# omid-arhami/topolow

Hardware: AMD Instinct MI355X
Metric: relaxation iterations/sec (NxN pairs) (higher is better)
Workload: dtype f32

## Files before the change

### topolow_amd/csrc/relax_symm.h

```cpp
#pragma once

#include <hip/hip_runtime.h>
#include <algorithm>
#include <type_traits>
#include <vector>
#include "relax_common.h"

namespace topolow {

#ifndef TOPOLOW_SYM_MINW
#define TOPOLOW_SYM_MINW 2
#endif
constexpr int kSymRows = 64;
constexpr int kSymCols = 32;
constexpr int kSymTileWords = kSymRows * kSymCols;
constexpr int kSymWaves = 4;

template <int DIM> struct SymRec { static constexpr int W = (DIM + 2 + 3) & ~3; };

struct SymUnit {
  int tile_row;
  int j0, j1;
  int tile0;
};

TL_HD inline long long sym_tile_index(int R, int J, int TC) { return (long long)R * TC - (long long)R * (R - 1) + (J - 2 * R); }
TL_HD inline size_t sym_word_in_tile(int r, int c) {
  const int a = r >> 3, p = (r & 7) >> 1, e = r & 1, b = c >> 2, h = (c & 3) >> 1, f = c & 1;
  return (size_t)((((4 * h + p) * 64) + a + 8 * b) * 4 + 2 * (f ^ (a & 1)) + e);
}

struct SymRun {
  int u0, u1;
  SymUnit first;
};
struct SymPlan {
  std::vector<SymUnit> units;
  std::vector<int> wave_first;
  std::vector<int2> row_units;
  std::vector<SymRun> runs() const {
    std::vector<SymRun> r(wave_first.size() - 1);
    for (size_t w = 0; w + 1 < wave_first.size(); ++w) {
      r[w].u0 = wave_first[w];
      r[w].u1 = wave_first[w + 1];
      r[w].first = r[w].u0 < r[w].u1 ? units[r[w].u0] : SymUnit{0, 0, 0, 0};
    }
    return r;
  }
};
inline SymPlan relax_symm_plan(int npad, int n_waves, long long t0 = 0, long long t1 = -1, int* r_first = nullptr,
                               int* r_last = nullptr) {
  SymPlan P;
  const int TR = npad / kSymRows, TC = npad / kSymCols;
  if (t1 < 0) t1 = (long long)TR * (TR + 1);
  const long long total = t1 - t0;
  int rf = -1, rl = -1;
  for (int R = 0; R < TR; ++R) {
    const long long a = sym_tile_index(R, 2 * R, TC), b = a + (TC - 2 * R);
    if (b > t0 && a < t1) { if (rf < 0) rf = R; rl = R; }
  }
  if (r_first) *r_first = rf;
  if (r_last) *r_last = rl;
  P.wave_first.assign(n_waves + 1, 0);
  if (rf < 0) return P;
  P.row_units.resize(rl - rf + 1);
  long long done = 0;
  int w = 0;
  long long w_end = (total * (w + 1) + n_waves - 1) / n_waves;
  for (int R = rf; R <= rl; ++R) {
    P.row_units[R - rf].x = (int)P.units.size();
    const long long row0 = sym_tile_index(R, 2 * R, TC);
    int j = 2 * R + (int)std::max<long long>(0, t0 - row0);
    const int j_end = 2 * R + (int)std::min<long long>(TC - 2 * R, t1 - row0);
    while (j < j_end) {
      while (done >= w_end && w + 1 < n_waves) {
        ++w;
        P.wave_first[w] = (int)P.units.size();
        w_end = (total * (w + 1) + n_waves - 1) / n_waves;
// ... 113 lines not shown
  bool sp0, sp1;
  if constexpr (THR) {
    const symf2 e0 = t - r;
    auto decide = [](uint32_t w, float e) {
      const uint32_t flip = (w << 30) & 0x80000000u;
      const int32_t some = (int32_t)(((w >> 1) | w) << 31) >> 31;
      const uint32_t q = ((f32_bits(e) ^ flip) & (uint32_t)some) | (0x3f800000u & ~(uint32_t)some);
      return bits_f32(q) > 0.0f;
    };
    sp0 = decide(w0, e0.x);
    sp1 = decide(w1, e0.y);
  } else {
    sp0 = __builtin_amdgcn_classf(bits_f32(w0), 0x1f8);
    sp1 = __builtin_amdgcn_classf(bits_f32(w1), 0x1f8);
  }
  const symf2 e = t - r;
  const symf2 inv2 = inv * inv;
  const symf2 u = {sp0 ? e.x : inv2.x, sp1 ? e.y : inv2.y};
  const symf2 base = u * inv;
  const symf2 mr = {sp0 ? ks2.x : cg2.x, sp1 ? ks2.y : cg2.y};
  const symf2 coef = base * mr;
#pragma unroll
  for (int d = 0; d < DIM; ++d) racc2[d] = __builtin_elementwise_fma(dx[d], coef, racc2[d]);
  const symf2 mc = {sp0 ? ksc : cgc, sp1 ? ksc : cgc};
  const symf2 cc = base * mc;
#pragma unroll
  for (int d = 0; d < DIM; ++d)
    cacc2[d] = FIRST ? dx[d] * cc : __builtin_elementwise_fma(dx[d], cc, cacc2[d]);
  if constexpr (ERR) {
    const symf2 a = {sp0 ? fabsf(e.x) : 0.0f, sp1 ? fabsf(e.y) : 0.0f};
    err2 += a;
    if constexpr (CNT) cnt_wave += (sp0 ? 1u : 0u) + (sp1 ? 1u : 0u);
  }
}

template <int DIM, bool ANYTHR, bool ERR>
__global__ __launch_bounds__(64 * kSymWaves, TOPOLOW_SYM_MINW) void symm_sweep_kernel(
    const uint32_t* __restrict__ enc, const float* __restrict__ rec, const SymUnit* __restrict__ units,
    const SymRun* __restrict__ runs, float* __restrict__ rowpart, float* __restrict__ colpart, int npad,
    const RunState* st, double* __restrict__ part_sum, unsigned long long* __restrict__ part_cnt,
    unsigned long long fixed_cnt, int col_row0) {
  if (st != nullptr && st->stopped) return;
#ifdef TOPOLOW_SYM_STAMPS
  const unsigned long long stamp_c0 = __builtin_amdgcn_s_memtime(), stamp_r0 = __builtin_amdgcn_s_memrealtime();
#endif
  constexpr int W = SymRec<DIM>::W;
  constexpr int kRecVec = W / 4;
  constexpr int kTileVec = kSymCols * kRecVec;
  constexpr int kLdsVec = kTileVec + kSymCols / 4;
  __shared__ uint4 lds[kSymWaves][2][kLdsVec];
  auto lds_slot = [](int q) { return q + (q / (4 * kRecVec)); };
  const int lane = threadIdx.x & 63;
  const int wave = __builtin_amdgcn_readfirstlane(threadIdx.x >> 6);
  const int a = lane & 7, b = lane >> 3;

  const int gw = blockIdx.x * kSymWaves + wave;
  const SymRun run = runs[gw];
  const int u_begin = __builtin_amdgcn_readfirstlane(run.u0);
  const int u_end = __builtin_amdgcn_readfirstlane(run.u1);
  typedef unsigned int u32x4 __attribute__((ext_vector_type(4)));
  const __amdgpu_buffer_rsrc_t rec_rsrc = __builtin_amdgcn_make_buffer_rsrc(const_cast<float*>(rec), 0, npad * W * 4, 0x00020000);
  for (int u = u_begin; u < u_end; ++u) {
    const SymUnit U = u == u_begin ? run.first : units[u];
    const int R = __builtin_amdgcn_readfirstlane(U.tile_row);
    const int J0 = __builtin_amdgcn_readfirstlane(U.j0), J1 = __builtin_amdgcn_readfirstlane(U.j1);
    const int slot = u;
    const int tile0 = __builtin_amdgcn_readfirstlane(U.tile0);

    symf2 pi2[4][DIM], ks2[4], cg2[4], racc2[4][DIM];
    {
      const uint4* rr = reinterpret_cast<const uint4*>(rec + (size_t)(R * kSymRows + 8 * a) * W);
#pragma unroll
      for (int p = 0; p < 4; ++p) {
        float f[2][W];
#pragma unroll
        for (int e = 0; e < 2; ++e)
#pragma unroll
          for (int v = 0; v < kRecVec; ++v) {
            const uint4 q = rr[(2 * p + e) * kRecVec + v];
            f[e][4 * v + 0] = __builtin_bit_cast(float, q.x);
            f[e][4 * v + 1] = __builtin_bit_cast(float, q.y);
            f[e][4 * v + 2] = __builtin_bit_cast(float, q.z);
            f[e][4 * v + 3] = __builtin_bit_cast(float, q.w);
          }
#pragma unroll
        for (int d = 0; d < DIM; ++d) {
          pi2[p][d] = (symf2){f[0][d], f[1][d]};
          racc2[p][d] = (symf2){0.0f, 0.0f};
        }
        ks2[p] = (symf2){f[0][DIM], f[1][DIM]};
        cg2[p] = (symf2){f[0][DIM + 1], f[1][DIM + 1]};
      }
    }
    const __amdgpu_buffer_rsrc_t rsrc = __builtin_amdgcn_make_buffer_rsrc(
        const_cast<uint32_t*>(enc) + (size_t)tile0 * kSymTileWords, 0, (J1 - J0) * kSymTileWords * 4, 0x00020000);
    const __amdgpu_buffer_rsrc_t col_rsrc = __builtin_amdgcn_make_buffer_rsrc(colpart + (size_t)(R - col_row0) * npad * DIM, 0, npad * DIM * 4, 0x00020000);
    const int col_off = a < 2 ? (4 * b + a) * DIM * 4 : 0x40000000;
    const int swap = a & 1;
    auto request = [&](int J, int h, u32x4 (&dst)[4]) {
#pragma unroll
      for (int p = 0; p < 4; ++p)
        dst[p] = __builtin_amdgcn_raw_buffer_load_b128(rsrc, lane * 16 + ((J - J0) * 8 + 4 * h + p) * 1024, 0, 0);
    };
    u32x4 wa[4], wb[4];
    request(J0, 0, wa);
    const uint4* recv = reinterpret_cast<const uint4*>(rec);
    if (lane < kTileVec) lds[wave][J0 & 1][lds_slot(lane)] = recv[(size_t)J0 * kTileVec + lane];
    if constexpr (kTileVec > 64) if (lane + 64 < kTileVec) lds[wave][J0 & 1][lds_slot(lane + 64)] = recv[(size_t)J0 * kTileVec + lane + 64];

    symf2 err2 = {0.0f, 0.0f};
    float err_unit = 0.0f;
    unsigned cnt_wave = 0, cnt_unit2 = 0;
    auto read_rec = [&](int J, int idx, float (&f)[W]) {
      const int col = idx ^ swap;
      const uint4* cp = &lds[wave][J & 1][4 * b * kRecVec + b];
#pragma unroll
      for (int v = 0; v < kRecVec; ++v) {
        const uint4 q = cp[col * kRecVec + v];
        f[4 * v + 0] = __builtin_bit_cast(float, q.x);
        f[4 * v + 1] = __builtin_bit_cast(float, q.y);
        f[4 * v + 2] = __builtin_bit_cast(float, q.z);
        f[4 * v + 3] = __builtin_bit_cast(float, q.w);
      }
    };
    float f_first[W];
    read_rec(J0, 0, f_first);
#pragma unroll 1
    for (int J = J0; J < J1; ++J) {
      const int Jn = J + 1 < J1 ? J + 1 : J;
      request(J, 1, wb);
      u32x4 rn0 = {0, 0, 0, 0}, rn1 = {0, 0, 0, 0};
      rn0 = __builtin_amdgcn_raw_buffer_load_b128(rec_rsrc, (Jn * kTileVec + lane) * 16, 0, 0);
      if constexpr (kTileVec > 64) rn1 = __builtin_amdgcn_raw_buffer_load_b128(rec_rsrc, (Jn * kTileVec + lane + 64) * 16, 0, 0);
      __builtin_amdgcn_sched_barrier(0);

      const bool diag = J < 2 * R + 2;
      float fq[4][W];
#pragma unroll
      for (int q = 0; q < W; ++q) fq[0][q] = f_first[q];
      auto half = [&](auto hc, const u32x4 (&wc)[4]) {
        constexpr int h = decltype(hc)::value;
        symf2 cacc2[2][DIM];
#pragma unroll
        for (int c = 0; c < 2; ++c) {
          if (2 * h + c + 1 < 4) {
            read_rec(J, 2 * h + c + 1, fq[2 * h + c + 1]);
            __builtin_amdgcn_sched_barrier(0);
          }
          const float (&f)[W] = fq[2 * h + c];
          float pc[DIM];
#pragma unroll
          for (int d = 0; d < DIM; ++d) pc[d] = f[d];
          const float ksc = f[DIM], cgc = f[DIM + 1];
#pragma unroll
          for (int p = 0; p < 4; ++p) {
            const uint32_t w0 = c == 0 ? wc[p].x : wc[p].z, w1 = c == 0 ? wc[p].y : wc[p].w;
            if (p == 0)
              sym_pair<DIM, ANYTHR, ERR, ANYTHR, true>(pc, ksc, cgc, pi2[p], ks2[p], cg2[p], w0, w1, racc2[p], cacc2[c], err2, cnt_wave);
            else
              sym_pair<DIM, ANYTHR, ERR, ANYTHR, false>(pc, ksc, cgc, pi2[p], ks2[p], cg2[p], w0, w1, racc2[p], cacc2[c], err2, cnt_wave);
          }
// ... 60 lines not shown
#pragma unroll
      for (int m = 32; m >= 1; m >>= 1) s += __shfl_xor(s, m, 64);
      if constexpr (ANYTHR) {
#pragma unroll
        for (int m = 32; m >= 1; m >>= 1) cnt_unit2 += __shfl_xor(cnt_unit2, m, 64);
      }
      if (lane == 0) {
        part_sum[slot] = s;
        part_cnt[slot] = ANYTHR ? (unsigned long long)cnt_unit2 : (slot == 0 ? fixed_cnt : 0ull);
      }
    }
  }
#ifdef TOPOLOW_SYM_STAMPS
  if (lane == 0 && g_sym_stamps != nullptr) {
    g_sym_stamps[4 * gw] = __builtin_amdgcn_s_memtime() - stamp_c0;
    g_sym_stamps[4 * gw + 1] = stamp_r0;
    g_sym_stamps[4 * gw + 2] = __builtin_amdgcn_s_memrealtime();
    unsigned hw_id, xcc_id;
    asm volatile("s_getreg_b32 %0, hwreg(HW_REG_HW_ID)" : "=s"(hw_id));
    asm volatile("s_getreg_b32 %0, hwreg(HW_REG_XCC_ID)" : "=s"(xcc_id));
    g_sym_stamps[4 * gw + 3] = ((unsigned long long)xcc_id << 32) | hw_id;
  }
#endif
}

template <int DIM, typename real> struct SymReal;
template <int DIM> struct SymReal<DIM, float> {
  static constexpr int W = SymRec<DIM>::W;
  __device__ static float ks(double k, float g) { return (float)(2.0 * k) / (4.0f * g + (float)k); }
  __device__ static float cg(double c_rep, float g) { return (float)(0.5 * c_rep) / g; }
  __device__ static float far(int) { return kFarF32; }
};

#ifndef TL_APPLY_PARTS
#define TL_APPLY_PARTS 16
#endif
constexpr int kSymApplyParts = TL_APPLY_PARTS;
template <int DIM, typename real>
__global__ __launch_bounds__(32 * kSymApplyParts) void symm_apply_kernel(
    const real* __restrict__ rec, real* __restrict__ rec_next, real* __restrict__ pos_out, const float* __restrict__ gplus,
    const real* __restrict__ rowpart, const real* __restrict__ colpart, const int2* __restrict__ row_units, int n,
    int npad, double k_next, double c_rep, int iter1, RunState* st, int rr_stages = 0, int rr_stage = 0) {
  if (st != nullptr && st->stopped) return;
  using T = SymReal<DIM, real>;
  constexpr int W = T::W;
  constexpr int kWavesA = kSymApplyParts / 2;
  __shared__ real red[kWavesA][kSymCols][DIM];
  const int R = blockIdx.x >> 1;
  const int part = threadIdx.x >> 5, pt = threadIdx.x & 31;
  const int i = blockIdx.x * kSymCols + pt;
  real acc[DIM];
#pragma unroll
  for (int d = 0; d < DIM; ++d) acc[d] = 0;
  int rp0 = 0, rp1 = R;
  if (rr_stages > 0) sym_rr_above(npad / kSymRows, rr_stages, rr_stage, R, rp0, rp1);
  for (int Rp = rp0 + part; Rp < rp1; Rp += kSymApplyParts) {
    const real* src = colpart + ((size_t)Rp * npad + i) * DIM;
#pragma unroll
    for (int d = 0; d < DIM; ++d) acc[d] += src[d];
  }
  const int2 ru = row_units[R];
  const int row_in_tile = i - R * kSymRows;
  for (int q = part; q < ru.y; q += kSymApplyParts) {
    const real* src = rowpart + ((size_t)(ru.x + q) * kSymRows + row_in_tile) * DIM;
#pragma unroll
    for (int d = 0; d < DIM; ++d) acc[d] -= src[d];
  }
#pragma unroll
  for (int d = 0; d < DIM; ++d) {
    if constexpr (std::is_same<real, float>::value) acc[d] += __shfl_xor(acc[d], 32, 64);
    else acc[d] += T::lane_xor(acc[d], 32);
  }
  const int wave = threadIdx.x >> 6;
  if ((threadIdx.x & 32) == 0) {
#pragma unroll
    for (int d = 0; d < DIM; ++d) red[wave][pt][d] = acc[d];
  }
  __syncthreads();
  if (part == 0 && i < n) {
    bool finite = true;
    real out[DIM];
#pragma unroll
    for (int d = 0; d < DIM; ++d) {
      real t = red[0][pt][d];
#pragma unroll
      for (int p = 1; p < kWavesA; ++p) t += red[p][pt][d];
      out[d] = rec[(size_t)i * W + d] + t;
      finite = finite && isfinite(out[d]);
      pos_out[(size_t)i * DIM + d] = out[d];
      rec_next[(size_t)i * W + d] = out[d];
    }
    const real g = (real)gplus[i];
    rec_next[(size_t)i * W + DIM] = T::ks(k_next, g);
    rec_next[(size_t)i * W + DIM + 1] = T::cg(c_rep, g);
    if (!finite && st != nullptr) atomicMin(&st->first_nonfinite, iter1);
  }
}

template <int DIM, typename real>
__global__ __launch_bounds__(256) void symm_records_kernel(const real* __restrict__ pos, const float* __restrict__ gplus,
                                                          real* __restrict__ rec, int n, int npad, double k, double c_rep) {
  using T = SymReal<DIM, real>;
  constexpr int W = T::W;
  const int i = blockIdx.x * blockDim.x + threadIdx.x;
  if (i >= npad) return;
  real* r = rec + (size_t)i * W;
  if (i < n) {
#pragma unroll
    for (int d = 0; d < DIM; ++d) r[d] = pos[(size_t)i * DIM + d];
    const real g = (real)gplus[i];
    r[DIM] = T::ks(k, g);
    r[DIM + 1] = T::cg(c_rep, g);
  } else {
#pragma unroll
    for (int d = 0; d < DIM; ++d) r[d] = T::far(d);
    r[DIM] = 0;
    r[DIM + 1] = 0;
  }
#pragma unroll
  for (int d = DIM + 2; d < W; ++d) r[d] = 0;
}

__global__ __launch_bounds__(256) void symm_tiles_kernel(const uint32_t* const* __restrict__ src, const int* __restrict__ row0,
                                                        int n_src, int ld, uint32_t* __restrict__ tenc, int TC,
                                                        long long t_first) {
  const long long t = t_first + blockIdx.x;
  int R = 0;
  {
    const double b = (double)TC + 1.0;
    const double disc = b * b - 4.0 * (double)t;
    R = (int)((b - sqrt(disc > 0.0 ? disc : 0.0)) * 0.5);
    while (R > 0 && (long long)R * TC - (long long)R * (R - 1) > t) --R;
    while ((long long)(R + 1) * TC - (long long)(R + 1) * R <= t) ++R;
  }
  const int J = 2 * R + (int)(t - ((long long)R * TC - (long long)R * (R - 1)));
  uint32_t* dst = tenc + (size_t)blockIdx.x * kSymTileWords;
  const int rows = row0[n_src];
#pragma unroll
  for (int q = 0; q < kSymTileWords / 256; ++q) {
    const int cell = threadIdx.x + q * 256;
    const int r = cell >> 5, c = cell & 31;
    const int row = R * kSymRows + r, col = J * kSymCols + c;
    uint32_t w = kInfWord;
    if (row < rows && col < ld) {
      int blk = 0;
      while (blk + 1 < n_src && row >= row0[blk + 1]) ++blk;
      w = src[blk][enc_index(row - row0[blk], col, ld)];
    }
    const int a = r >> 3, p = (r & 7) >> 1, e = r & 1, b = c >> 2, h = (c & 3) >> 1, f = c & 1;
    dst[(((4 * h + p) * 64) + a + 8 * b) * 4 + 2 * (f ^ (a & 1)) + e] = w;
  }
}


template <int DIM>
__global__ __launch_bounds__(32 * 32) void symm_partial_kernel(
    const float* __restrict__ rowpart, const float* __restrict__ colpart, const int2* __restrict__ row_units, int r_first,
    int r_last, int n, int npad, float* const* __restrict__ inbox, const int* __restrict__ own0, int n_own, int slot,
    const RunState* st) {
  if (st != nullptr && st->stopped) return;
  __shared__ float red[32][kSymCols][DIM];
  const int R = blockIdx.x >> 1;
  const int part = threadIdx.x >> 5, pt = threadIdx.x & 31;
  const int i = blockIdx.x * kSymCols + pt;
  float acc[DIM];
#pragma unroll
  for (int d = 0; d < DIM; ++d) acc[d] = 0.0f;
  const int r_stop = R < r_last + 1 ? R : r_last + 1;
  for (int Rp = r_first + part; Rp < r_stop; Rp += 32) {
    const float* src = colpart + ((size_t)(Rp - r_first) * npad + i) * DIM;
#pragma unroll
    for (int d = 0; d < DIM; ++d) acc[d] += src[d];
  }
  if (R >= r_first && R <= r_last) {
    const int2 ru = row_units[R - r_first];
    const int row_in_tile = i - R * kSymRows;
    for (int q = part; q < ru.y; q += 32) {
      const float* src = rowpart + ((size_t)(ru.x + q) * kSymRows + row_in_tile) * DIM;
#pragma unroll
      for (int d = 0; d < DIM; ++d) acc[d] -= src[d];
    }
  }
#pragma unroll
  for (int d = 0; d < DIM; ++d) red[part][pt][d] = acc[d];
  __syncthreads();
  if (part == 0 && i < n) {
    int q = 0;
    while (q + 1 < n_own && i >= own0[q + 1]) ++q;
    float* dst = inbox[q] + ((size_t)slot * npad + i) * DIM;
#pragma unroll
    for (int d = 0; d < DIM; ++d) {
      float t = red[0][pt][d];
#pragma unroll
      for (int p = 1; p < 32; ++p) t += red[p][pt][d];
      dst[d] = t;
    }
  }
}

template <int DIM>
__global__ __launch_bounds__(256) void symm_owner_apply_kernel(
    const float* __restrict__ pos_in, float* __restrict__ pos_out, const float* __restrict__ inbox, int n_slots, int npad,
    int row_begin, int row_end, float* const* __restrict__ push, int n_push, int iter1, RunState* st) {
  if (st != nullptr && st->stopped) return;
  const int i = row_begin + blockIdx.x * blockDim.x + threadIdx.x;
  if (i >= row_end) return;
  bool finite = true;
  float out[DIM];
#pragma unroll
  for (int d = 0; d < DIM; ++d) {
    float t = 0.0f;
    for (int b = 0; b < n_slots; ++b) t += inbox[((size_t)b * npad + i) * DIM + d];
    out[d] = pos_in[(size_t)i * DIM + d] + t;
    finite = finite && isfinite(out[d]);
    pos_out[(size_t)i * DIM + d] = out[d];
  }
  for (int q = 0; q < n_push; ++q) {
    float* dst = push[q];
#pragma unroll
// ... 7 lines not shown
```

### topolow_amd/csrc/topolow_relax.hip

```cpp

#include <hip/hip_runtime.h>

#include <chrono>
#include <cstdarg>
#include <cstdio>
#include <algorithm>
#include <cstring>
#include <cstdlib>
#include <array>
#include <atomic>
#include <deque>
#include <mutex>
#include <string>
#include <memory>
#include <thread>
#include <vector>

#include "../../include/topolow_relax.h"
#include "relax_common.h"
#include "relax_host.h"
#include "relax_kernels.h"
#include "relax_fold.h"
#include "relax_gs.h"
#include "relax_tilegs.h"
// ... 144 lines not shown
  struct SymState {
    bool allowed = false;
    int min_n = 0;
    bool ready = false;
    int npad = 0, tiles = 0, grid = 0;
    DevBuf<uint32_t> tenc;
    DevBuf<unsigned char> rec[2], rowpart, colpart;
    int rec_cur = 0, rec_iter = -1;
    DevBuf<float> tdelta;
    bool delta_ready = false;
    struct Plan {
      DevBuf<SymUnit> units;
      DevBuf<SymRun> runs;
      DevBuf<int2> row_units;
      int n_units = 0;
      void load(const SymPlan& hp) {
        const std::vector<SymRun> hr = hp.runs();
        n_units = (int)hp.units.size();
        units.alloc(std::max<size_t>(hp.units.size(), 1));
        runs.alloc(hr.size());
        row_units.alloc(std::max<size_t>(hp.row_units.size(), 1));
        if (!hp.units.empty())
          HIP_TRY(hipMemcpy(units.p, hp.units.data(), hp.units.size() * sizeof(SymUnit), hipMemcpyHostToDevice));
        HIP_TRY(hipMemcpy(runs.p, hr.data(), hr.size() * sizeof(SymRun), hipMemcpyHostToDevice));
        if (!hp.row_units.empty())
          HIP_TRY(hipMemcpy(row_units.p, hp.row_units.data(), hp.row_units.size() * sizeof(int2), hipMemcpyHostToDevice));
      }
      void release() { units.release(); runs.release(); row_units.release(); n_units = 0; }
    };
    Plan plan;
    std::vector<Plan> rr[4];
    bool whole = false;
    bool two_stage = true;
    int rr_min_tiles = 5;
    DevBuf<const uint32_t*> src_tab;
    DevBuf<int> src_row0;
    bool seg_ready = false;
    bool seg_thr = false;
    int seg_first = 0, seg_last = -1;
    int seg_slots = 0;
    int seg_slot = 0;
    bool seg_caller = false;
    DevBuf<float> inbox;
    DevBuf<float*> inbox_tab;
    DevBuf<int> own0;
    std::vector<const void*> seg_peers;

    void release() {
      tenc.release(); rec[0].release(); rec[1].release(); rowpart.release(); colpart.release();
      tdelta.release(); delta_ready = false;
      plan.release();
      for (auto& v : rr) v.clear();
      src_tab.release(); src_row0.release();
      inbox.release(); inbox_tab.release(); own0.release();
    }
  } sym;
  int fused_parts = 0;
  bool profiling = false;
  std::vector<std::pair<hipEvent_t, hipEvent_t>> prof_stage, prof_stage_err, prof_check;
  std::vector<std::pair<hipEvent_t, hipEvent_t>> prof_sym, prof_sym_err;

  size_t real_size() const { return precision == TOPOLOW_PRECISION_F64 ? 8 : 4; }
  int rows() const { return row_end - row_begin; }
  int pos_rows() const { return (n + 3) & ~3; }

  ~topolow_session() {
// ... 484 lines not shown
}

template <int DIM>
void sym_prepare(topolow_session* s) {
  sym_build<DIM>(s, {s->enc.p}, {0, s->rows()}, s->any_threshold, 0, -1);
  s->sym.ready = true;
  s->sym.seg_ready = false;
}

bool sym_available(topolow_session* s) {
  if (s->sym.ready) return true;
  try {
    TL_DISPATCH_SYM(s->dim, sym_prepare, s);
  } catch (const HipError&) {
    (void)hipGetLastError();
    s->sym.release();
    s->sym.ready = false;
    s->sym.allowed = false;
  }
  return s->sym.ready;
}

template <int DIM>
void sym_records(topolow_session* s, const void* pin, void* rec, double k) {
  sym_real(s, [&](auto r) {
    using real = decltype(r);
    hipLaunchKernelGGL((symm_records_kernel<DIM, real>), dim3((s->sym.npad + 255) / 256), dim3(256), 0, s->stream,
                       (const real*)pin, s->gplus.p, (real*)rec, s->n, s->sym.npad, k, s->c_rep);
  });
}

template <int DIM>
void sym_sweep(topolow_session* s, const SymPlanDev& plan, const void* rec, bool thr, bool err,
               unsigned long long block_cells, int col_row0) {
  auto& y = s->sym;
  sym_real(s, [&](auto r) {
    using real = decltype(r);
    sym_sweep_instance<DIM, real>(thr, err, [&](auto kern) {
      if constexpr (std::is_same<real, double>::value)
        hipLaunchKernelGGL(kern, dim3(y.grid), dim3(64 * kSymWaves), 0, s->stream, y.tenc.p, (const double*)rec,
                           plan.units.p, plan.runs.p, (double*)y.rowpart.p, (double*)y.colpart.p, y.npad, s->state.p,
                           col_row0, y.tdelta.p, s->part_sum.p, s->part_cnt.p, block_cells);
      else
        hipLaunchKernelGGL(kern, dim3(y.grid), dim3(64 * kSymWaves), 0, s->stream, y.tenc.p, (const float*)rec,
                           plan.units.p, plan.runs.p, (float*)y.rowpart.p, (float*)y.colpart.p, y.npad, s->state.p,
                           s->part_sum.p, s->part_cnt.p, block_cells, col_row0);
    });
  });
}

template <int DIM>
void sym_apply(topolow_session* s, const SymPlanDev& plan, const void* rec, void* rec_next, void* pout, double k_next,
               int iter, int rr_stages, int rr_stage) {
  auto& y = s->sym;
  sym_real(s, [&](auto r) {
    using real = decltype(r);
    hipLaunchKernelGGL((symm_apply_kernel<DIM, real>), dim3(y.npad / kSymCols), dim3(32 * kSymApplyParts), 0, s->stream,
                       (const real*)rec, (real*)rec_next, (real*)pout, s->gplus.p, (const real*)y.rowpart.p,
                       (const real*)y.colpart.p, plan.row_units.p, s->n, y.npad, k_next, s->c_rep, iter + 1, s->state.p,
                       rr_stages, rr_stage);
  });
}

bool sym_rr_stages_ok(int S) { return S == 2 || S == 4 || S == 8; }
int sym_rr_log2(int S) { return S == 2 ? 1 : (S == 4 ? 2 : 3); }

bool sym_rr_available(topolow_session* s, int S) {
  auto& y = s->sym;
  if (!sym_rr_stages_ok(S) || !y.whole) return false;
  const int TR = y.npad / kSymRows;
  if (TR < 2 * S) return false;
  if ((long long)TR * (TR + 1) / S < (long long)y.rr_min_tiles * y.grid * kSymWaves) return false;
  const int lg = sym_rr_log2(S);
  if (!y.rr[lg].empty()) return true;
  std::vector<SymPlanDev> plans(S);
  for (int st = 0; st < S; ++st) {
    const SymPlan hp = relax_symm_plan_rows(y.npad, y.grid * kSymWaves, [&](int R, int& j0, int& j1) { sym_rr_row(TR, S, st, R, j0, j1); });
    if (hp.units.size() * kSymRows * s->dim * s->real_size() > y.rowpart.n) return false;
    plans[st].load(hp);
  }
  y.rr[lg] = std::move(plans);
  return true;
}

template <int DIM>
void sym_iteration(topolow_session* s, const void* pin, void* pout, int iter, double k, bool err, int S = 0, int st = 0,
                   bool last = true) {
  auto& y = s->sym;
  const SymPlanDev& plan = S == 0 ? y.plan : y.rr[sym_rr_log2(S)][st];
  ProfScope prof(s, S > 0 ? &s->prof_stage : err ? &s->prof_sym_err : &s->prof_sym);
  if (err && s->precision == TOPOLOW_PRECISION_F64 && !y.delta_ready)
    throw HipError{TOPOLOW_ERR_UNSUPPORTED, "symmetric sweep (f64): no delta tiles for a fused check"};
  if (y.rec_iter != iter) {
    for (int b = 0; b < 2; ++b)
      sym_records<DIM>(s, pin, y.rec[b].p, k);
    y.rec_cur = 0;
  }
  sym_sweep<DIM>(s, plan, y.rec[y.rec_cur].p, s->any_threshold, err, S == 0 ? s->block_cells : 0ull, 0);
  sym_apply<DIM>(s, plan, y.rec[y.rec_cur].p, y.rec[y.rec_cur ^ 1].p, pout, last ? k * (1.0 - s->cooling) : k, iter, S, st);
  HIP_TRY(hipGetLastError());
  y.rec_cur ^= 1;
  y.rec_iter = last ? iter + 1 : iter;
  if (err) s->fused_parts = plan.n_units;
  s->stage_launches += 1;
}

enum class SymForm { kRowOwner, kSweep, kStages };
SymForm sym_form(topolow_session* s, int n_stages) {
  if (n_stages == 1) return sym_eligible(s) && sym_available(s) ? SymForm::kSweep : SymForm::kRowOwner;
  return s->sym.two_stage && sym_rr_stages_ok(n_stages) && sym_eligible(s) && sym_available(s) &&
                 sym_rr_available(s, n_stages)
             ? SymForm::kStages
             : SymForm::kRowOwner;
}

int iteration_stages(const topolow_session* s, int iter, double k) {
  return slab_geom(s->n, s->fixed_stages > 0 ? s->fixed_stages : slab_stages_at(iter, k, s->dim)).n_stages;
}

bool check_after(const topolow_session* s, int iter) { return (iter + 1) % s->check_freq == 0 || iter == s->n_iter - 1; }

struct IterPlan {
  SlabGeom geo;
  SymForm form;
  int order[8];
};
IterPlan plan_iteration(topolow_session* s, int iter, double k) {
  IterPlan p;
  p.geo = slab_geom(s->n, iteration_stages(s, iter, k));
  p.form = sym_form(s, p.geo.n_stages);
  if (p.form == SymForm::kStages) sym_rr_order(s->seed, iter, p.geo.n_stages, p.order);
// ... 86 lines not shown
  y.seg_caller = false;
  sym_inbox<DIM>(s, P, row0);
  HIP_TRY(hipStreamSynchronize(s->stream));
  y.seg_peers = peers;
}

void sym_sharded_prepare(std::vector<topolow_session*>& ss) {
  const int P = (int)ss.size();
  for (topolow_session* s : ss) {
    HIP_TRY(hipSetDevice(s->device));
    HIP_TRY(hipDeviceSynchronize());
  }
  for (int b = 0; b < P; ++b) TL_DISPATCH_SYM(ss[b]->dim, sym_sharded_build, ss, b);
  for (int b = 0; b < P; ++b) {
    topolow_session* s = ss[b];
    HIP_TRY(hipSetDevice(s->device));
    for (topolow_session* q : ss)
      if (q != s && q->rows() > 0)
        HIP_TRY(hipMemcpy(s->gplus.p + q->row_begin, q->gplus.p + q->row_begin, (size_t)q->rows() * sizeof(float),
                          hipMemcpyDeviceToDevice));
    std::vector<float*> tab;
    for (topolow_session* q : ss) tab.push_back(q->sym.inbox.p);
    s->sym.inbox_tab.alloc(P);
    HIP_TRY(hipMemcpy(s->sym.inbox_tab.p, tab.data(), P * sizeof(float*), hipMemcpyHostToDevice));
    s->sym.seg_ready = true;
  }
}

template <int DIM>
void sym_sharded_sweep(topolow_session* s, const void* pin, int iter, double k, bool err) {
  auto& y = s->sym;
  ProfScope prof(s, err ? &s->prof_sym_err : &s->prof_sym);
  sym_records<DIM>(s, pin, y.rec[0].p, k);
  if (y.tiles > 0) sym_sweep<DIM>(s, y.plan, y.rec[0].p, y.seg_thr, err, s->block_cells, y.seg_first);
  hipLaunchKernelGGL(symm_partial_kernel<DIM>, dim3(y.npad / kSymCols), dim3(32 * 32), 0, s->stream, (const float*)y.rowpart.p,
                     (const float*)y.colpart.p, y.plan.row_units.p, y.seg_first, y.seg_last, s->n, y.npad, y.inbox_tab.p,
                     y.own0.p, y.seg_slots, y.seg_slot, s->state.p);
  HIP_TRY(hipGetLastError());
  if (err) s->fused_parts = y.plan.n_units;
  (void)iter;
  s->stage_launches += 1;
}

template <int DIM>
void sym_owner_apply(topolow_session* s, const void* pin, void* pout, int row_begin, int row_end, const void* push,
                     int n_push, int iter) {
  auto& y = s->sym;
  hipLaunchKernelGGL(symm_owner_apply_kernel<DIM>, dim3((row_end - row_begin + 255) / 256), dim3(256), 0, s->stream,
                     (const float*)pin, (float*)pout, y.inbox.p, y.seg_slots, y.npad, row_begin, row_end,
                     (float* const*)push, n_push, iter + 1, s->state.p);
  HIP_TRY(hipGetLastError());
}

template <int DIM>
void sym_segment_build(topolow_session* s, int segment, int P, const uint32_t* d_rows, int row_first, int n_rows,
                       bool any_thr) {
  auto& y = s->sym;
  const SymSegment g = sym_segment(s->n, segment, P);
  if (g.r_first >= 0 && (row_first > g.r_first * kSymRows ||
                         row_first + n_rows < std::min<long long>(s->n, (long long)(g.r_last + 1) * kSymRows)))
    throw HipError{TOPOLOW_ERR_BAD_ARGUMENT, "symm_segment_build: d_rows does not hold the rows of the segment's tiles"};
  sym_build<DIM>(s, {d_rows}, {row_first, row_first + n_rows}, any_thr, g.t0, g.t1);
  if (y.seg_first < 0) { y.seg_first = 0; y.seg_last = -1; }
  y.ready = false;
  y.seg_thr = any_thr;
  y.seg_slots = 1;
  y.seg_slot = 0;
// ... 134 lines not shown
    set_err(errbuf, errlen, "bad row block [%d,%d) for n=%d", row_begin, row_end, n);
    return TOPOLOW_ERR_BAD_ARGUMENT;
  }
  topolow_session* s = nullptr;
  const int rc = guarded(errbuf, errlen, [&] {
    const int dev = select_device(device);
    s = new topolow_session();
    s->device = dev;
    s->n = n;
    s->dim = kernel_dim(ndim);
    s->udim = ndim;
    s->row_begin = row_begin;
    s->row_end = row_end;
    s->ld = (n + kEncLdAlign - 1) & ~(kEncLdAlign - 1);
    s->precision = precision == TOPOLOW_PRECISION_F64 ? TOPOLOW_PRECISION_F64
                                                      : TOPOLOW_PRECISION_F32;
    HIP_TRY(hipStreamCreateWithFlags(&s->own_stream, hipStreamNonBlocking));
    s->stream = s->own_stream;
    HIP_TRY(hipStreamCreateWithFlags(&s->check_stream, hipStreamNonBlocking));
    HIP_TRY(hipEventCreateWithFlags(&s->ev_iter_done, hipEventDisableTiming));
    HIP_TRY(hipEventCreateWithFlags(&s->ev_check_done, hipEventDisableTiming));
    const char* serial = getenv("TOPOLOW_SERIAL_CHECKS");
    s->serial_checks = serial != nullptr && serial[0] == '1';
    const char* fuse = getenv("TOPOLOW_FUSE_CHECKS");
    s->fuse_checks = !(fuse != nullptr && fuse[0] == '0');
    const char* symm = getenv("TOPOLOW_SYMMETRIC");
    s->sym.allowed = !(symm != nullptr && symm[0] == '0');
    const char* symm_min = getenv("TOPOLOW_SYMMETRIC_MIN_N");
    s->sym.min_n = symm_min != nullptr ? atoi(symm_min) : kSymMinPoints;
    const char* symm2 = getenv("TOPOLOW_SYMMETRIC_TWO_STAGE");
    s->sym.two_stage = !(symm2 != nullptr && symm2[0] == '0');
    const char* rr_min = getenv("TOPOLOW_SYMMETRIC_STAGE_MIN_TILES");
    if (rr_min != nullptr) s->sym.rr_min_tiles = std::max(0, atoi(rr_min));
    s->enc.alloc((size_t)((s->rows() + kEncRowAlign - 1) / kEncRowAlign * kEncRowAlign) * s->ld);
    const size_t pos_bytes = (size_t)s->pos_rows() * s->dim * s->real_size();
    for (auto& b : s->pos) b.alloc(pos_bytes);
    s->best.alloc(pos_bytes);
    s->state.alloc(1);
    HIP_TRY(hipHostMalloc((void**)&s->mailbox, sizeof(RunState), hipHostMallocMapped));
    std::memset(s->mailbox, 0, sizeof(RunState));
    HIP_TRY(hipHostGetDevicePointer((void**)&s->mailbox_dev, s->mailbox, 0));
  });
  if (rc != TOPOLOW_OK) { delete s; return rc; }
  *out = s;
  return TOPOLOW_OK;
}

void topolow_session_destroy(topolow_session* s) {
  if (!s) return;
  (void)hipSetDevice(s->device);
  if (s->stream) (void)hipStreamSynchronize(s->stream);
  if (s->check_stream) (void)hipStreamSynchronize(s->check_stream);
#ifdef TOPOLOW_TUNING
  g_stamps.dump();
#endif
  delete s;
}

int topolow_session_set_relabel(topolow_session* s, uint64_t seed, char* errbuf, size_t errlen) {
  if (!s) return TOPOLOW_ERR_BAD_ARGUMENT;
  if (s->gplus.p || s->part_sum.p) {
    set_err(errbuf, errlen, "the relabelling must be chosen before targets, edges or positions are loaded");
    return TOPOLOW_ERR_BAD_ARGUMENT;
  }
  return guarded(errbuf, errlen, [&] {
    HIP_TRY(hipSetDevice(s->device));
// ... 1336 lines not shown
```

Before: 17020.

## Batch strip loads in apply/partial kernels and hoist stop-flag loads

```diff
diff --git a/topolow_amd/csrc/relax_symm.h b/topolow_amd/csrc/relax_symm.h
--- a/topolow_amd/csrc/relax_symm.h
+++ b/topolow_amd/csrc/relax_symm.h
@@ -2,6 +2,7 @@
 
 #include <hip/hip_runtime.h>
 #include <algorithm>
+#include <cstddef>
 #include <type_traits>
 #include <vector>
 #include "relax_common.h"
@@ -223,6 +224,17 @@
     err2 += a;
     if constexpr (CNT) cnt_wave += (sp0 ? 1u : 0u) + (sp1 ? 1u : 0u);
   }
+}
+
+__device__ __forceinline__ int sym_load_stopped(const RunState* st) {
+  const __amdgpu_buffer_rsrc_t r = __builtin_amdgcn_make_buffer_rsrc(const_cast<RunState*>(st), 0, st != nullptr ? (int)sizeof(RunState) : 0, 0x00020000);
+  return (int)__builtin_amdgcn_raw_buffer_load_b32(r, (int)offsetof(RunState, stopped), 0, 0);
+}
+__device__ __forceinline__ int2 sym_load_row_units(const int2* row_units, int idx, bool have) {
+  typedef unsigned int u32x2 __attribute__((ext_vector_type(2)));
+  const __amdgpu_buffer_rsrc_t r = __builtin_amdgcn_make_buffer_rsrc(const_cast<int2*>(row_units), 0, have ? (idx + 1) * (int)sizeof(int2) : 0, 0x00020000);
+  const u32x2 q = __builtin_amdgcn_raw_buffer_load_b64(r, idx * (int)sizeof(int2), 0, 0);
+  return int2{(int)q.x, (int)q.y};
 }
 
 template <int DIM, bool ANYTHR, bool ERR>
@@ -444,6 +456,29 @@
   __device__ static float far(int) { return kFarF32; }
 };
 
+constexpr int kSymApplyBatch = 8;
+template <int DIM, typename real>
+__device__ __forceinline__ void sym_strips_load(real (&v)[kSymApplyBatch][DIM], const real* __restrict__ base, size_t stride,
+                                                int s0, int step, int end, int spare) {
+#pragma unroll
+  for (int b = 0; b < kSymApplyBatch; ++b) {
+    const int s = s0 + b * step;
+    const real* src = base + (size_t)(s < end ? s : spare) * stride;
+#pragma unroll
+    for (int d = 0; d < DIM; ++d) v[b][d] = src[d];
+  }
+  __builtin_amdgcn_sched_barrier(0);
+}
+template <int DIM, bool SUB, typename real>
+__device__ __forceinline__ void sym_strips_add(real (&acc)[DIM], const real (&v)[kSymApplyBatch][DIM], int s0, int step, int end) {
+#pragma unroll
+  for (int b = 0; b < kSymApplyBatch; ++b) {
+    const bool on = s0 + b * step < end;
+#pragma unroll
+    for (int d = 0; d < DIM; ++d) acc[d] = on ? (SUB ? acc[d] - v[b][d] : acc[d] + v[b][d]) : acc[d];
+  }
+}
+
 #ifndef TL_APPLY_PARTS
 #define TL_APPLY_PARTS 16
 #endif
@@ -453,30 +488,43 @@
     const real* __restrict__ rec, real* __restrict__ rec_next, real* __restrict__ pos_out, const float* __restrict__ gplus,
     const real* __restrict__ rowpart, const real* __restrict__ colpart, const int2* __restrict__ row_units, int n,
     int npad, double k_next, double c_rep, int iter1, RunState* st, int rr_stages = 0, int rr_stage = 0) {
-  if (st != nullptr && st->stopped) return;
   using T = SymReal<DIM, real>;
   constexpr int W = T::W;
   constexpr int kWavesA = kSymApplyParts / 2;
+  constexpr int kStep = kSymApplyParts * kSymApplyBatch;
   __shared__ real red[kWavesA][kSymCols][DIM];
   const int R = blockIdx.x >> 1;
   const int part = threadIdx.x >> 5, pt = threadIdx.x & 31;
   const int i = blockIdx.x * kSymCols + pt;
-  real acc[DIM];
-#pragma unroll
-  for (int d = 0; d < DIM; ++d) acc[d] = 0;
+  const int stopped = sym_load_stopped(st);
+  const int2 ru = sym_load_row_units(row_units, R, true);
   int rp0 = 0, rp1 = R;
   if (rr_stages > 0) sym_rr_above(npad / kSymRows, rr_stages, rr_stage, R, rp0, rp1);
-  for (int Rp = rp0 + part; Rp < rp1; Rp += kSymApplyParts) {
-    const real* src = colpart + ((size_t)Rp * npad + i) * DIM;
-#pragma unroll
-    for (int d = 0; d < DIM; ++d) acc[d] += src[d];
-  }
-  const int2 ru = row_units[R];
-  const int row_in_tile = i - R * kSymRows;
-  for (int q = part; q < ru.y; q += kSymApplyParts) {
-    const real* src = rowpart + ((size_t)(ru.x + q) * kSymRows + row_in_tile) * DIM;
-#pragma unroll
-    for (int d = 0; d < DIM; ++d) acc[d] -= src[d];
+  const real* cbase = colpart + (size_t)i * DIM;
+  const size_t cstride = (size_t)npad * DIM;
+  real v[kSymApplyBatch][DIM];
+  sym_strips_load<DIM>(v, cbase, cstride, rp0 + part, kSymApplyParts, rp1, rp0);
+  const bool mover = part == 0 && i < n;
+  real p_old[DIM], g = 1;
+  if (mover) {
+#pragma unroll
+    for (int d = 0; d < DIM; ++d) p_old[d] = rec[(size_t)i * W + d];
+    g = (real)gplus[i];
+  }
+  asm volatile("" ::: "memory");
+  if (stopped) return;
+  real acc[DIM];
+#pragma unroll
+  for (int d = 0; d < DIM; ++d) acc[d] = 0;
+  sym_strips_add<DIM, false>(acc, v, rp0 + part, kSymApplyParts, rp1);
+  for (int Rp = rp0 + part + kStep; Rp < rp1; Rp += kStep) {
+    sym_strips_load<DIM>(v, cbase, cstride, Rp, kSymApplyParts, rp1, rp0);
+    sym_strips_add<DIM, false>(acc, v, Rp, kSymApplyParts, rp1);
+  }
+  const real* rbase = rowpart + ((size_t)ru.x * kSymRows + (i - R * kSymRows)) * DIM;
+  for (int q = part; q < ru.y; q += kStep) {
+    sym_strips_load<DIM>(v, rbase, (size_t)kSymRows * DIM, q, kSymApplyParts, ru.y, q);
+    sym_strips_add<DIM, true>(acc, v, q, kSymApplyParts, ru.y);
   }
 #pragma unroll
   for (int d = 0; d < DIM; ++d) {
@@ -489,7 +537,7 @@
     for (int d = 0; d < DIM; ++d) red[wave][pt][d] = acc[d];
   }
   __syncthreads();
-  if (part == 0 && i < n) {
+  if (mover) {
     bool finite = true;
     real out[DIM];
 #pragma unroll
@@ -497,12 +545,11 @@
       real t = red[0][pt][d];
 #pragma unroll
       for (int p = 1; p < kWavesA; ++p) t += red[p][pt][d];
-      out[d] = rec[(size_t)i * W + d] + t;
+      out[d] = p_old[d] + t;
       finite = finite && isfinite(out[d]);
       pos_out[(size_t)i * DIM + d] = out[d];
       rec_next[(size_t)i * W + d] = out[d];
     }
-    const real g = (real)gplus[i];
     rec_next[(size_t)i * W + DIM] = T::ks(k_next, g);
     rec_next[(size_t)i * W + DIM + 1] = T::cg(c_rep, g);
     if (!finite && st != nullptr) atomicMin(&st->first_nonfinite, iter1);
@@ -570,33 +617,38 @@
     const float* __restrict__ rowpart, const float* __restrict__ colpart, const int2* __restrict__ row_units, int r_first,
     int r_last, int n, int npad, float* const* __restrict__ inbox, const int* __restrict__ own0, int n_own, int slot,
     const RunState* st) {
-  if (st != nullptr && st->stopped) return;
+  const int stopped = sym_load_stopped(st);
   __shared__ float red[32][kSymCols][DIM];
+  constexpr int kStep = 32 * kSymApplyBatch;
   const int R = blockIdx.x >> 1;
   const int part = threadIdx.x >> 5, pt = threadIdx.x & 31;
   const int i = blockIdx.x * kSymCols + pt;
+  const bool own_row = R >= r_first && R <= r_last;
+  const int2 ru = sym_load_row_units(row_units, own_row ? R - r_first : 0, own_row);
+  const int r_stop = R < r_last + 1 ? R : r_last + 1;
+  const int n_above = r_stop - r_first;
+  const float* cbase = colpart + (size_t)i * DIM;
+  const size_t cstride = (size_t)npad * DIM;
+  float v[kSymApplyBatch][DIM];
+  sym_strips_load<DIM>(v, cbase, cstride, part, 32, n_above, 0);
+  const int c_end = stopped ? 0 : n_above, r_end = stopped ? 0 : ru.y;
   float acc[DIM];
 #pragma unroll
   for (int d = 0; d < DIM; ++d) acc[d] = 0.0f;
-  const int r_stop = R < r_last + 1 ? R : r_last + 1;
-  for (int Rp = r_first + part; Rp < r_stop; Rp += 32) {
-    const float* src = colpart + ((size_t)(Rp - r_first) * npad + i) * DIM;
-#pragma unroll
-    for (int d = 0; d < DIM; ++d) acc[d] += src[d];
-  }
-  if (R >= r_first && R <= r_last) {
-    const int2 ru = row_units[R - r_first];
-    const int row_in_tile = i - R * kSymRows;
-    for (int q = part; q < ru.y; q += 32) {
-      const float* src = rowpart + ((size_t)(ru.x + q) * kSymRows + row_in_tile) * DIM;
-#pragma unroll
-      for (int d = 0; d < DIM; ++d) acc[d] -= src[d];
-    }
+  sym_strips_add<DIM, false>(acc, v, part, 32, c_end);
+  for (int q = part + kStep; q < c_end; q += kStep) {
+    sym_strips_load<DIM>(v, cbase, cstride, q, 32, c_end, 0);
+    sym_strips_add<DIM, false>(acc, v, q, 32, c_end);
+  }
+  const float* rbase = rowpart + ((size_t)ru.x * kSymRows + (i - R * kSymRows)) * DIM;
+  for (int q = part; q < r_end; q += kStep) {
+    sym_strips_load<DIM>(v, rbase, (size_t)kSymRows * DIM, q, 32, r_end, q);
+    sym_strips_add<DIM, true>(acc, v, q, 32, r_end);
   }
 #pragma unroll
   for (int d = 0; d < DIM; ++d) red[part][pt][d] = acc[d];
   __syncthreads();
-  if (part == 0 && i < n) {
+  if (part == 0 && i < n && !stopped) {
     int q = 0;
     while (q + 1 < n_own && i >= own0[q + 1]) ++q;
     float* dst = inbox[q] + ((size_t)slot * npad + i) * DIM;
```

After: 16330. -4.1%, worse.

## Prioritize waves with more remaining tiles and prefetch next unit descriptor

Applied to the files above, without the earlier changes.

```diff
diff --git a/topolow_amd/csrc/relax_symm.h b/topolow_amd/csrc/relax_symm.h
--- a/topolow_amd/csrc/relax_symm.h
+++ b/topolow_amd/csrc/relax_symm.h
@@ -30,9 +30,11 @@
   return (size_t)((((4 * h + p) * 64) + a + 8 * b) * 4 + 2 * (f ^ (a & 1)) + e);
 }
 
-struct SymRun {
+struct alignas(32) SymRun {
   int u0, u1;
   SymUnit first;
+  int tiles;
+  int reserved;
 };
 struct SymPlan {
   std::vector<SymUnit> units;
@@ -44,6 +46,9 @@
       r[w].u0 = wave_first[w];
       r[w].u1 = wave_first[w + 1];
       r[w].first = r[w].u0 < r[w].u1 ? units[r[w].u0] : SymUnit{0, 0, 0, 0};
+      r[w].tiles = 0;
+      for (int u = r[w].u0; u < r[w].u1; ++u) r[w].tiles += units[u].j1 - units[u].j0;
+      r[w].reserved = 0;
     }
     return r;
   }
@@ -230,8 +235,20 @@
     const uint32_t* __restrict__ enc, const float* __restrict__ rec, const SymUnit* __restrict__ units,
     const SymRun* __restrict__ runs, float* __restrict__ rowpart, float* __restrict__ colpart, int npad,
     const RunState* st, double* __restrict__ part_sum, unsigned long long* __restrict__ part_cnt,
-    unsigned long long fixed_cnt, int col_row0) {
-  if (st != nullptr && st->stopped) return;
+    unsigned long long fixed_cnt, int col_row0, int prio) {
+  const int wave = __builtin_amdgcn_readfirstlane(threadIdx.x >> 6);
+  const int gw = blockIdx.x * kSymWaves + wave;
+  const SymRun run = runs[gw];
+  int stopped = st->stopped;
+  if constexpr (ERR)
+    asm("" : "+s"(stopped) : "s"(run.u0), "s"(run.u1), "s"(run.first.tile_row), "s"(run.first.j0), "s"(run.first.j1),
+        "s"(run.first.tile0), "s"(run.tiles), "s"(enc), "s"(rec), "s"(units),
+        "s"(rowpart), "s"(colpart), "s"(npad), "s"(col_row0), "s"(prio), "s"(part_sum), "s"(part_cnt), "s"(fixed_cnt));
+  else
+    asm("" : "+s"(stopped) : "s"(run.u0), "s"(run.u1), "s"(run.first.tile_row), "s"(run.first.j0), "s"(run.first.j1),
+        "s"(run.first.tile0), "s"(run.tiles), "s"(enc), "s"(rec), "s"(units),
+        "s"(rowpart), "s"(colpart), "s"(npad), "s"(col_row0), "s"(prio));
+  if (stopped) return;
 #ifdef TOPOLOW_SYM_STAMPS
   const unsigned long long stamp_c0 = __builtin_amdgcn_s_memtime(), stamp_r0 = __builtin_amdgcn_s_memrealtime();
 #endif
@@ -242,19 +259,21 @@
   __shared__ uint4 lds[kSymWaves][2][kLdsVec];
   auto lds_slot = [](int q) { return q + (q / (4 * kRecVec)); };
   const int lane = threadIdx.x & 63;
-  const int wave = __builtin_amdgcn_readfirstlane(threadIdx.x >> 6);
   const int a = lane & 7, b = lane >> 3;
 
-  const int gw = blockIdx.x * kSymWaves + wave;
-  const SymRun run = runs[gw];
   const int u_begin = __builtin_amdgcn_readfirstlane(run.u0);
   const int u_end = __builtin_amdgcn_readfirstlane(run.u1);
   typedef unsigned int u32x4 __attribute__((ext_vector_type(4)));
   const __amdgpu_buffer_rsrc_t rec_rsrc = __builtin_amdgcn_make_buffer_rsrc(const_cast<float*>(rec), 0, npad * W * 4, 0x00020000);
+  int left = __builtin_amdgcn_readfirstlane(run.tiles);
+  const int lv3 = (3 * left) >> 2, lv2 = left >> 1, lv1 = left >> 2;
+  SymUnit U_next = run.first;
   for (int u = u_begin; u < u_end; ++u) {
-    const SymUnit U = u == u_begin ? run.first : units[u];
+    const SymUnit U = U_next;
+    U_next = units[u + 1 < u_end ? u + 1 : u];
     const int R = __builtin_amdgcn_readfirstlane(U.tile_row);
     const int J0 = __builtin_amdgcn_readfirstlane(U.j0), J1 = __builtin_amdgcn_readfirstlane(U.j1);
+    __builtin_assume(J0 < J1);
     const int slot = u;
     const int tile0 = __builtin_amdgcn_readfirstlane(U.tile0);
 
@@ -318,6 +337,13 @@
     read_rec(J0, 0, f_first);
 #pragma unroll 1
     for (int J = J0; J < J1; ++J) {
+      if (prio) {
+        if (left > lv3) __builtin_amdgcn_s_setprio(3);
+        else if (left > lv2) __builtin_amdgcn_s_setprio(2);
+        else if (left > lv1) __builtin_amdgcn_s_setprio(1);
+        else __builtin_amdgcn_s_setprio(0);
+      }
+      --left;
       const int Jn = J + 1 < J1 ? J + 1 : J;
       request(J, 1, wb);
       u32x4 rn0 = {0, 0, 0, 0}, rn1 = {0, 0, 0, 0};
@@ -453,12 +479,16 @@
     const real* __restrict__ rec, real* __restrict__ rec_next, real* __restrict__ pos_out, const float* __restrict__ gplus,
     const real* __restrict__ rowpart, const real* __restrict__ colpart, const int2* __restrict__ row_units, int n,
     int npad, double k_next, double c_rep, int iter1, RunState* st, int rr_stages = 0, int rr_stage = 0) {
-  if (st != nullptr && st->stopped) return;
+  const int R = blockIdx.x >> 1;
+  const int2 ru = row_units[R];
+  int stopped = st->stopped;
+  asm("" : "+s"(stopped) : "s"(ru.x), "s"(ru.y), "s"(rec), "s"(rowpart), "s"(colpart), "s"(n), "s"(npad), "s"(rr_stages), "s"(rr_stage),
+      "s"(rec_next), "s"(pos_out), "s"(gplus), "s"(k_next), "s"(c_rep));
+  if (stopped) return;
   using T = SymReal<DIM, real>;
   constexpr int W = T::W;
   constexpr int kWavesA = kSymApplyParts / 2;
   __shared__ real red[kWavesA][kSymCols][DIM];
-  const int R = blockIdx.x >> 1;
   const int part = threadIdx.x >> 5, pt = threadIdx.x & 31;
   const int i = blockIdx.x * kSymCols + pt;
   real acc[DIM];
@@ -471,7 +501,6 @@
 #pragma unroll
     for (int d = 0; d < DIM; ++d) acc[d] += src[d];
   }
-  const int2 ru = row_units[R];
   const int row_in_tile = i - R * kSymRows;
   for (int q = part; q < ru.y; q += kSymApplyParts) {
     const real* src = rowpart + ((size_t)(ru.x + q) * kSymRows + row_in_tile) * DIM;
@@ -505,7 +534,7 @@
     const real g = (real)gplus[i];
     rec_next[(size_t)i * W + DIM] = T::ks(k_next, g);
     rec_next[(size_t)i * W + DIM + 1] = T::cg(c_rep, g);
-    if (!finite && st != nullptr) atomicMin(&st->first_nonfinite, iter1);
+    if (!finite) atomicMin(&st->first_nonfinite, iter1);
   }
 }
 
diff --git a/topolow_amd/csrc/topolow_relax.hip b/topolow_amd/csrc/topolow_relax.hip
--- a/topolow_amd/csrc/topolow_relax.hip
+++ b/topolow_amd/csrc/topolow_relax.hip
@@ -200,6 +200,7 @@
     std::vector<Plan> rr[4];
     bool whole = false;
     bool two_stage = true;
+    bool prio = true;
     int rr_min_tiles = 5;
     DevBuf<const uint32_t*> src_tab;
     DevBuf<int> src_row0;
@@ -750,7 +751,7 @@
 
 template <int DIM>
 void sym_sweep(topolow_session* s, const SymPlanDev& plan, const void* rec, bool thr, bool err,
-               unsigned long long block_cells, int col_row0) {
+               unsigned long long block_cells, int col_row0, bool prio) {
   auto& y = s->sym;
   sym_real(s, [&](auto r) {
     using real = decltype(r);
@@ -762,7 +763,7 @@
       else
         hipLaunchKernelGGL(kern, dim3(y.grid), dim3(64 * kSymWaves), 0, s->stream, y.tenc.p, (const float*)rec,
                            plan.units.p, plan.runs.p, (float*)y.rowpart.p, (float*)y.colpart.p, y.npad, s->state.p,
-                           s->part_sum.p, s->part_cnt.p, block_cells, col_row0);
+                           s->part_sum.p, s->part_cnt.p, block_cells, col_row0, prio && y.prio ? 1 : 0);
     });
   });
 }
@@ -814,7 +815,7 @@
       sym_records<DIM>(s, pin, y.rec[b].p, k);
     y.rec_cur = 0;
   }
-  sym_sweep<DIM>(s, plan, y.rec[y.rec_cur].p, s->any_threshold, err, S == 0 ? s->block_cells : 0ull, 0);
+  sym_sweep<DIM>(s, plan, y.rec[y.rec_cur].p, s->any_threshold, err, S == 0 ? s->block_cells : 0ull, 0, true);
   sym_apply<DIM>(s, plan, y.rec[y.rec_cur].p, y.rec[y.rec_cur ^ 1].p, pout, last ? k * (1.0 - s->cooling) : k, iter, S, st);
   HIP_TRY(hipGetLastError());
   y.rec_cur ^= 1;
@@ -967,7 +968,8 @@
   auto& y = s->sym;
   ProfScope prof(s, err ? &s->prof_sym_err : &s->prof_sym);
   sym_records<DIM>(s, pin, y.rec[0].p, k);
-  if (y.tiles > 0) sym_sweep<DIM>(s, y.plan, y.rec[0].p, y.seg_thr, err, s->block_cells, y.seg_first);
+  if (y.tiles > 0) sym_sweep<DIM>(s, y.plan, y.rec[0].p, y.seg_thr, err, s->block_cells, y.seg_first,
+                                  false);
   hipLaunchKernelGGL(symm_partial_kernel<DIM>, dim3(y.npad / kSymCols), dim3(32 * 32), 0, s->stream, (const float*)y.rowpart.p,
                      (const float*)y.colpart.p, y.plan.row_units.p, y.seg_first, y.seg_last, s->n, y.npad, y.inbox_tab.p,
                      y.own0.p, y.seg_slots, y.seg_slot, s->state.p);
@@ -1168,6 +1170,8 @@
     s->sym.two_stage = !(symm2 != nullptr && symm2[0] == '0');
     const char* rr_min = getenv("TOPOLOW_SYMMETRIC_STAGE_MIN_TILES");
     if (rr_min != nullptr) s->sym.rr_min_tiles = std::max(0, atoi(rr_min));
+    const char* sym_prio = getenv("TOPOLOW_SYM_PRIO");
+    s->sym.prio = !(sym_prio != nullptr && sym_prio[0] == '0');
     s->enc.alloc((size_t)((s->rows() + kEncRowAlign - 1) / kEncRowAlign * kEncRowAlign) * s->ld);
     const size_t pos_bytes = (size_t)s->pos_rows() * s->dim * s->real_size();
     for (auto& b : s->pos) b.alloc(pos_bytes);
```

Result: faster. 16820 before, 17790 after, median of 6 (+5.7%).
